# Corleno/Nonstationary_Multivariate_Gaussian_Process

Hardware: AMD Instinct MI355X
Metric: log-posterior evals/sec (N=2048, D=3 nonseparable GP) (higher is better)
Workload: dtype f64

## Files before the change

nonstationary_multivariate_gaussian_process_amd/csrc/nmgp_chol.hip:

```cpp
#include "nmgp_internal.h"
#include <cstring>

namespace nmgpk {

static inline int cdiv_c(long long a, long long b) { return (int)((a + b - 1) / b); }

typedef double v4d __attribute__((ext_vector_type(4)));

#define SY_BM 128
#define SY_BK 16
#define SY_LD (SY_BM + 16)
#define SY_SB 8

__device__ __forceinline__ int clamp_row_pair(int r, int rows) {
    int rc = r < rows - 1 ? r : rows - 2;
    return rc < 0 ? 0 : rc;
}

__device__ __forceinline__ double fast_recip(double p) {
    double x = __builtin_amdgcn_rcp(p);
    double e = fma(-p, x, 1.0);
    x = fma(x, e, x);
    e = fma(-p, x, 1.0);
    x = fma(x, e, x);
    return x;
}

template <int KC, int GC>
__device__ __forceinline__ void potf2_step(double (&a)[16], double (*colbuf)[64], double* pivs, int nb,
                                           int* __restrict__ info, int goff, int r, int g, int tid) {
    constexpr int c = 4 * KC + GC;
    constexpr int NKC = (GC == 3) ? KC + 1 : KC;
    constexpr int NGC = (GC == 3) ? 0 : GC + 1;
    if (c >= nb) return;
    const double* cb = colbuf[c & 1];
    const double piv = cb[c];
    const double mine = cb[r];
    double t[16];
#pragma unroll
    for (int kk = KC; kk < 16; ++kk) t[kk] = cb[4 * kk + g];
    if (tid == 0) {
        pivs[c] = piv;
        if (!(piv > 0.0)) atomicCAS(info, 0, goff + c + 1);
    }
    const double pinv = fast_recip(piv);
    const double f = mine * pinv;
    if (c + 1 < 64) {
        if (NKC < 16) {
            const int cc = 4 * NKC + g;
            const double upd = fma(-f, t[NKC < 16 ? NKC : 15], a[NKC < 16 ? NKC : 15]);
            const bool on = (g == NGC) && (cc <= r);
            if (NKC < 16) a[NKC < 16 ? NKC : 15] = on ? upd : a[NKC < 16 ? NKC : 15];
            if (g == NGC) colbuf[(c + 1) & 1][r] = a[NKC < 16 ? NKC : 15];
        }
        __syncthreads();
    }
#pragma unroll
    for (int kk = KC; kk < 16; ++kk) {
        const int cc = 4 * kk + g;
        const double upd = fma(-f, t[kk], a[kk]);
        bool on = (kk > KC || g > GC) && (cc <= r);
        if (kk == NKC) on = on && (g != NGC);
        a[kk] = on ? upd : a[kk];
    }
}

template <int KC>
__device__ __forceinline__ void potf2_steps4(double (&a)[16], double (*colbuf)[64], double* pivs, int nb,
                                             int* __restrict__ info, int goff, int r, int g, int tid) {
    potf2_step<KC, 0>(a, colbuf, pivs, nb, info, goff, r, g, tid);
    potf2_step<KC, 1>(a, colbuf, pivs, nb, info, goff, r, g, tid);
    potf2_step<KC, 2>(a, colbuf, pivs, nb, info, goff, r, g, tid);
    potf2_step<KC, 3>(a, colbuf, pivs, nb, info, goff, r, g, tid);
}

__device__ __forceinline__ void potf2_body(double* __restrict__ A, int lda, int nb, int* __restrict__ info, int goff, int tid,
                                           double (*colbuf)[64], double* pivs) {
    const int r = tid & 63, g = (tid >> 6) & 3;
    double a[16];
#pragma unroll
    for (int kk = 0; kk < 16; ++kk) {
        const int c = 4 * kk + g;
        double v = (r == c) ? 1.0 : 0.0;
        if (r < nb && c <= r) v = A[(size_t)c * lda + r];
        a[kk] = v;
    }
    if (tid < 64) pivs[tid] = 1.0;
    if (g == 0) colbuf[0][r] = a[0];
    __syncthreads();
#define PF(K) potf2_steps4<K>(a, colbuf, pivs, nb, info, goff, r, g, tid)
    PF(0); PF(1); PF(2); PF(3); PF(4); PF(5); PF(6); PF(7); PF(8); PF(9); PF(10); PF(11); PF(12); PF(13); PF(14); PF(15);
#undef PF
    __syncthreads();
#pragma unroll
    for (int kk = 0; kk < 16; ++kk) {
        const int c = 4 * kk + g;
        if (r < nb && c <= r) A[(size_t)c * lda + r] = a[kk] * rsqrt(pivs[c]);
    }
}

typedef double v2d __attribute__((ext_vector_type(2)));
typedef int v4i __attribute__((ext_vector_type(4)));

__device__ __forceinline__ void syrk_fused_first_block(double* lds, const v4d (&acc)[2][2][2], bool owner, int wj,
                                                       double* __restrict__ C, int ldc, int* __restrict__ info, int goff);

#define SY_SMEM (4 * SY_BK * SY_LD)
#define SCHUR_PATCH (32 * 33)
#define SY_SCHUR_SMEM (8 * SCHUR_PATCH + 6 * 256)
static_assert(SY_SCHUR_SMEM >= SY_SMEM && SY_SCHUR_SMEM * 8 * 2 <= 160 * 1024, "Schur epilogue LDS");

template <int M>
__device__ __forceinline__ double svc_schur_value(double sigma2, int a, int b, bool rc, const double* __restrict__ Lr, double il2,
                                                  const double* __restrict__ Lc, double kv, double nai, double gcb) {
    constexpr int UR = M <= 3 ? 8 : 1;
    const double gra = sigma2 * Lr[a * (a + 1) / 2] * il2;
    double s = 0.0;
#pragma unroll UR
    for (int q = 1; q <= b; ++q) s += Lr[a * (a + 1) / 2 + q] * Lc[b * (b + 1) / 2 + q];
    double v = kv * s;
    if (rc) v += sigma2 * ((a == b ? 1.0 : 0.0) + Lr[a * (a + 1) / 2] * Lr[b * (b + 1) / 2] * il2);
    v += gra * nai * gcb;
    return v;
}

template <int M, bool ALLB>
__device__ __forceinline__ void svc_schur_entries(const SchurEpi& e, double sigma2, int r, const double* __restrict__ Lr, double il2,
                                                  int c, double kv, double nai, const double* gc) {
    constexpr int T = M * (M + 1) / 2;
    constexpr int UR = M <= 3 ? 8 : 1;
    const size_t Ns = (size_t)e.N;
    const double* __restrict__ Lc = e.Lv + (size_t)c * T;
    const double lcc = M <= 4 ? 0.0 : Lc[0];
#pragma unroll UR
    for (int a = 1; a < M; ++a) {
#pragma unroll UR
        for (int b = 1; b <= (ALLB ? a : a - 1); ++b) {
            const double gcb = M <= 4 ? gc[b - 1] : sigma2 * Lc[b * (b + 1) / 2] / (lcc * lcc);
            e.S[((size_t)(b - 1) * Ns + c) * e.ld + ((size_t)(a - 1) * Ns + r)] =
                svc_schur_value<M>(sigma2, a, b, r == c, Lr, il2, Lc, kv, nai, gcb);
        }
    }
}

constexpr int svc_gstride(int M) { return M + 2; }

template <int M>
__device__ __forceinline__ void svc_schur_gtable(const SchurEpi& e, double* lds, int row0, int col0, int tid) {
    constexpr int T = M * (M + 1) / 2, GS = svc_gstride(M);
    if constexpr (M <= 4) {
        double* gt = lds + 8 * SCHUR_PATCH;
        if (tid < 256) {
            const int loc = tid < 128 ? col0 + tid : row0 + tid - 128;
            if (loc < e.N) {
                const double sigma2 = exp(e.tse[0]);
                const double* Lc = e.Lv + (size_t)loc * T;
                const double l00 = Lc[0];
#pragma unroll
                for (int b = 1; b < M; ++b) gt[tid * GS + b - 1] = sigma2 * Lc[b * (b + 1) / 2] / (l00 * l00);
                gt[tid * GS + M - 1] = 1.0 / (l00 * l00);
                gt[tid * GS + M] = e.x[loc];
                gt[tid * GS + M + 1] = e.ell[loc];
            }
        }
        __syncthreads();
    }
}

template <int M>
__device__ __forceinline__ void svc_schur_patch(const SchurEpi& e, double* P, const double* lds, int i0, int j0, int row0, int col0,
                                                int lane) {
    constexpr int T_ = M * (M + 1) / 2, GS = svc_gstride(M);
    constexpr int QU = M <= 3 ? 2 : 1;
    const int N = e.N;
    const size_t Ns = (size_t)N;
    const double sigma2 = exp(e.tse[0]);
    const double* gt = lds + 8 * SCHUR_PATCH;
    const int lo = lane & 31, hi = lane >> 5;
    __builtin_amdgcn_wave_barrier();
#pragma unroll
    for (int pass = 0; pass < 2; ++pass) {
        if (pass == 1 && M == 2) break;
        const int r = (pass == 0 ? i0 : j0) + lo;
        if (r < N) {
            const double* __restrict__ Lr = e.Lv + (size_t)r * T_;
            const double xr = e.x[r], lr = e.ell[r];
            const double xr2 = xr * xr, lr2 = lr * lr;
            const double l00 = Lr[0];
            const double il2 = 1.0 / (l00 * l00);
#pragma unroll QU
            for (int q = 0; q < 16; ++q) {
                const int o = 2 * q + hi;
                const int il = pass == 0 ? lo : o, jl = pass == 0 ? o : lo;
                const int c = (pass == 0 ? j0 : i0) + o;
                if (pass == 0 ? (c > r || c >= N) : (c <= r || c >= N)) continue;
                const double* gc = gt + (pass == 0 ? c - col0 : 128 + c - row0) * GS;
                if (pass == 1 && M == 3) {
                    e.S[(size_t)c * e.ld + (Ns + r)] = P[il * 33 + jl];
                    continue;
                }
                const double xc = M <= 4 ? gc[M] : e.x[c], lc = M <= 4 ? gc[M + 1] : e.ell[c];
                const double dist = (xr2 + xc * xc) - 2.0 * (xr * xc);
                const double Aa = lr2 + lc * lc;
                double kv = sqrt(2.0 * (lr * lc) / Aa) * exp(-dist / Aa);
                if (r == c) kv = NMGP_JITTER + kv;
                const double nai = P[il * 33 + jl];
                if (pass == 0) {
                    svc_schur_entries<M, true>(e, sigma2, r, Lr, il2, c, kv, nai, gc);
                    if (M == 3 && c < r) {
                        const double* Lc = e.Lv + (size_t)c * T_;
                        P[il * 33 + jl] = svc_schur_value<M>(sigma2, 2, 1, false, Lc, gc[M - 1], Lr, kv, nai, gt[(128 + r - row0) * GS]);
                    }
                } else {
                    svc_schur_entries<M, false>(e, sigma2, r, Lr, il2, c, kv, nai, gc);
                }
            }
        }
        __builtin_amdgcn_wave_barrier();
    }
}

template <int M>
__device__ __forceinline__ void svc_schur_yrow(const SchurEpi& e, int i) {
    constexpr int T = M * (M + 1) / 2;
    if (i >= e.N) return;
    const size_t Ns = (size_t)e.N;
    const int n1 = (M - 1) * e.N;
    const double sigma2 = exp(e.tse[0]);
    const double* Li = e.Lv + (size_t)i * T;
    const double l00 = Li[0];
    const double il2 = 1.0 / (l00 * l00);
    const double vi = e.y[i] / l00;
    const double r = vi - (sigma2 * il2) * e.u[i];
#pragma unroll
    for (int a = 1; a < M; ++a) e.S[((size_t)(a - 1) * Ns + i) * e.ld + n1] = e.y[(size_t)a * Ns + i] - Li[a * (a + 1) / 2] * r;
}

template <int SM = 0>
__device__ __forceinline__ void syrk_tile_fast(const double* __restrict__ A, int lda, double* __restrict__ C, int ldc, int K,
                                               int row0, int col0, bool diag, int kt0, bool beta0, int ncw, int yrow,
                                               int nyr, double* sA0, double* sB0, bool skip00 = false,
                                               int* __restrict__ finfo = nullptr, int fgoff = 0, bool mirror = false,
                                               int fresh0 = 0x7fffffff, const SchurEpi* se = nullptr) {
    constexpr int BK = 16;
    constexpr int SBUF = BK * SY_LD;
    const int tid = threadIdx.x, lane = tid & 63, w = tid >> 6;
    const int wi = w & 1, wj = w >> 1;
    const int l15 = lane & 15, l4 = lane >> 4;
    const int rp = tid & 63, cg = tid >> 6;
    const int offA = (cg * lda + row0 + 2 * rp) * 8, offB = (cg * lda + col0 + 2 * rp) * 8;
    const __amdgpu_buffer_rsrc_t rsrc = __builtin_amdgcn_make_buffer_rsrc((void*)A, 0, 0x7fffffff, 0x00020000);
    const int gstep = BK * lda * 8, ghalf = 8 * lda * 8;
    int soff = kt0 * gstep;
    const bool has_y = diag && yrow >= 0;
    const bool ywave = has_y && wi == 0 && wj >= 2;
    const int offY = ((tid & 15) * lda + yrow + (tid >> 4)) * 8;
    double* sY = sB0;
    v4i ra0, ra1, rb0, rb1;
    double ry = 0.0;
    auto gload = [&]() {
        ra0 = __builtin_amdgcn_raw_buffer_load_b128(rsrc, offA, soff, 0);
        ra1 = __builtin_amdgcn_raw_buffer_load_b128(rsrc, offA, soff + ghalf, 0);
        if (!diag) {
            rb0 = __builtin_amdgcn_raw_buffer_load_b128(rsrc, offB, soff, 0);
            rb1 = __builtin_amdgcn_raw_buffer_load_b128(rsrc, offB, soff + ghalf, 0);
        }
        if (has_y && tid < 16 * nyr) {
            typedef int v2i __attribute__((ext_vector_type(2)));
            const v2i t2 = __builtin_amdgcn_raw_buffer_load_b64(rsrc, offY, soff, 0);
            ry = __builtin_bit_cast(double, t2);
        }
        soff += gstep;
    };
    double* wA = sA0 + cg * SY_LD + 2 * rp;
    double* wB = sB0 + cg * SY_LD + 2 * rp;
    auto sstore = [&](int buf) {
        *reinterpret_cast<v4i*>(wA + buf * SBUF) = ra0;
        *reinterpret_cast<v4i*>(wA + buf * SBUF + 8 * SY_LD) = ra1;
        if (!diag) {
            *reinterpret_cast<v4i*>(wB + buf * SBUF) = rb0;
            *reinterpret_cast<v4i*>(wB + buf * SBUF + 8 * SY_LD) = rb1;
        }
        if (has_y && tid < 16 * nyr) sY[buf * 256 + tid] = ry;
    };
    const bool active = !(diag && (wi * 64 + 63 < wj * 32)) && (wj * 32 < ncw) && !(skip00 && wi == 0 && wj < 2);
    const int nk = K / BK;
    gload();
    v4d acc[2][2][2];
    if (active) {
        const int rw0 = __builtin_amdgcn_readfirstlane(row0 + wi * 64);
        const bool wload = !beta0 && rw0 < fresh0;
#pragma unroll
        for (int p = 0; p < 2; ++p) {
            const int i = row0 + wi * 64 + 32 * p + 2 * l15;
            const bool old = i < fresh0;
#pragma unroll
            for (int tj = 0; tj < 2; ++tj)
#pragma unroll
                for (int r = 0; r < 4; ++r) {
                    const int j = col0 + wj * 32 + 2 * (l4 + 4 * r) + tj;
                    double2 c = make_double2(0.0, 0.0);
                    if (wload && old) c = *reinterpret_cast<const double2*>(&C[(size_t)j * ldc + i]);
                    acc[p][0][tj][r] = -c.x;
                    acc[p][1][tj][r] = -c.y;
                }
        }
    }
    if (ywave) {
#pragma unroll
        for (int u = 0; u < 2; ++u)
#pragma unroll
            for (int t = 0; t < 2; ++t)
#pragma unroll
                for (int r = 0; r < 4; ++r) {
                    const int j = col0 + 64 * (wj - 2) + 32 * u + 2 * (l4 + 4 * r) + t;
                    acc[u][0][t][r] = (l15 < nyr && yrow + l15 < fresh0) ? -C[(size_t)j * ldc + yrow + l15] : 0.0;
                }
    }
    sstore(0);
    __syncthreads();
    const double* rA = sA0 + wi * 64 + 2 * l15 + l4 * SY_LD;
    const double* rB = (diag ? sA0 : sB0) + wj * 32 + 2 * l15 + l4 * SY_LD;
    auto compute = [&](int buf) {
        const double* tA = rA + buf * SBUF;
        const double* tB = rB + buf * SBUF;
        v2d fa[2], fb, na[2], nb;
        fa[0] = *reinterpret_cast<const v2d*>(tA);
        fa[1] = *reinterpret_cast<const v2d*>(tA + 32);
        fb = *reinterpret_cast<const v2d*>(tB);
#pragma unroll
        for (int kk = 0; kk < BK / 4; ++kk) {
            if (kk + 1 < BK / 4) {
                na[0] = *reinterpret_cast<const v2d*>(tA + (kk + 1) * 4 * SY_LD);
                na[1] = *reinterpret_cast<const v2d*>(tA + (kk + 1) * 4 * SY_LD + 32);
                nb = *reinterpret_cast<const v2d*>(tB + (kk + 1) * 4 * SY_LD);
            }
#pragma unroll
            for (int tj = 0; tj < 2; ++tj)
#pragma unroll
                for (int p = 0; p < 2; ++p)
#pragma unroll
                    for (int sx = 0; sx < 2; ++sx)
                        acc[p][sx][tj] = __builtin_amdgcn_mfma_f64_16x16x4f64(fb[tj], fa[p][sx], acc[p][sx][tj], 0, 0, 0);
            if (kk + 1 < BK / 4) {
                fa[0] = na[0];
                fa[1] = na[1];
                fb = nb;
            }
        }
    };
    const double* rY = sA0 + 64 * (wj - 2) + 2 * l15 + l4 * SY_LD;
    const int yz = (l15 < nyr) ? yrow + l15 - fresh0 - l4 : 0x7fffffff;
    auto compute_y = [&](int buf, int kb) {
        const double* tB = rY + buf * SBUF;
        const double* ty = sY + buf * 256 + l15 * 16 + l4;
#pragma unroll
        for (int kk = 0; kk < BK / 4; ++kk) {
            const v2d f0 = *reinterpret_cast<const v2d*>(tB + kk * 4 * SY_LD);
            const v2d f1 = *reinterpret_cast<const v2d*>(tB + kk * 4 * SY_LD + 32);
            const double yv = ty[4 * kk];
            const double fy = (kb + 4 * kk >= yz) ? yv : 0.0;
            acc[0][0][0] = __builtin_amdgcn_mfma_f64_16x16x4f64(f0[0], fy, acc[0][0][0], 0, 0, 0);
            acc[0][0][1] = __builtin_amdgcn_mfma_f64_16x16x4f64(f0[1], fy, acc[0][0][1], 0, 0, 0);
            acc[1][0][0] = __builtin_amdgcn_mfma_f64_16x16x4f64(f1[0], fy, acc[1][0][0], 0, 0, 0);
            acc[1][0][1] = __builtin_amdgcn_mfma_f64_16x16x4f64(f1[1], fy, acc[1][0][1], 0, 0, 0);
        }
    };
    for (int kt = kt0; kt < nk; kt += 2) {
        gload();
        if (active) compute(0);
        else if (ywave) compute_y(0, kt * BK);
        sstore(1);
        __syncthreads();
        if (kt + 2 < nk) gload();
        if (active) compute(1);
        else if (ywave) compute_y(1, kt * BK + BK);
        if (kt + 2 < nk) sstore(0);
        __syncthreads();
    }
    if constexpr (SM > 0) {
        svc_schur_gtable<SM>(*se, sA0, row0, col0, tid);
        if (active) {
            double* P = sA0 + w * SCHUR_PATCH;
#pragma unroll
            for (int p = 0; p < 2; ++p) {
#pragma unroll
                for (int sx = 0; sx < 2; ++sx)
#pragma unroll
                    for (int tj = 0; tj < 2; ++tj)
#pragma unroll
                        for (int r = 0; r < 4; ++r) P[(2 * l15 + sx) * 33 + 2 * (l4 + 4 * r) + tj] = -acc[p][sx][tj][r];
                svc_schur_patch<SM>(*se, P, sA0, row0 + wi * 64 + 32 * p, col0 + wj * 32, row0, col0, lane);
            }
        }
        if (diag && wj == 0) svc_schur_yrow<SM>(*se, row0 + wi * 64 + lane);
        return;
    }
    if (ywave && l15 < nyr) {
#pragma unroll
        for (int u = 0; u < 2; ++u)
#pragma unroll
            for (int t = 0; t < 2; ++t)
#pragma unroll
                for (int r = 0; r < 4; ++r) {
                    const int j = col0 + 64 * (wj - 2) + 32 * u + 2 * (l4 + 4 * r) + t;
                    C[(size_t)j * ldc + yrow + l15] = -acc[u][0][t][r];
                }
    }
    const bool fowner = finfo != nullptr && wi == 0 && wj < 2;
    if (active && !fowner) {
#pragma unroll
    for (int p = 0; p < 2; ++p)
#pragma unroll
        for (int tj = 0; tj < 2; ++tj)
#pragma unroll
            for (int r = 0; r < 4; ++r) {
                const int i = row0 + wi * 64 + 32 * p + 2 * l15;
                const int j = col0 + wj * 32 + 2 * (l4 + 4 * r) + tj;
                if (diag && j > i + 1) continue;
                double2 c;
                c.x = -acc[p][0][tj][r];
                c.y = -acc[p][1][tj][r];
                if (diag && j == i + 1) C[(size_t)j * ldc + i + 1] = c.y;
                else *reinterpret_cast<double2*>(&C[(size_t)j * ldc + i]) = c;
            }
    }
    if (mirror && active) {
        double* T = sA0 + w * (32 * 33);
        const int jl = lane & 31, ih = lane >> 5;
#pragma unroll
        for (int p = 0; p < 2; ++p) {
#pragma unroll
            for (int sx = 0; sx < 2; ++sx)
#pragma unroll
                for (int tj = 0; tj < 2; ++tj)
#pragma unroll
                    for (int r = 0; r < 4; ++r) T[(2 * l15 + sx) * 33 + 2 * (l4 + 4 * r) + tj] = -acc[p][sx][tj][r];
            const int rowm = col0 + wj * 32 + jl;
#pragma unroll
            for (int q = 0; q < 16; ++q) {
                const int il = 2 * q + ih;
                const int colm = row0 + wi * 64 + 32 * p + il;
                const double v = T[il * 33 + jl];
                if (colm > rowm) C[(size_t)colm * ldc + rowm] = v;
            }
        }
    }
    if (finfo != nullptr) syrk_fused_first_block(sA0, acc, fowner, wj, C, ldc, finfo, fgoff);
}

template <int NWJ, int BK, int SM = 0>
__device__ __forceinline__ void syrk_tile_body(const double* __restrict__ A, int lda, double* __restrict__ C, int ldc, int mrows,
                                               int ncols, int K, long long bstride, long long cstride, int ktri, int swz,
                                               int nbatch, int bx, int by, int bz0, double* sAb, double* sBb,
                                               int tri_row0 = 0x7fffffff, int tri_k0 = 0, int* __restrict__ finfo = nullptr,
                                               int fistride = 0, int fgoff = 0, const SchurEpi* sep = nullptr) {
    const int nyr = (ktri >> 2) & 31;
    const bool skipq = (ktri & 128) != 0;
    const bool mirror = (ktri & 512) != 0;
    const bool rowmajor = (ktri & 1024) != 0;
    const int yrow = nyr ? mrows : -1;
    (void)rowmajor;
    ktri &= 1;
    const int fresh0 = tri_row0 == 0x7fffffff ? 0x7fffffff : tri_row0 + tri_k0;
    constexpr int NT = 128 * NWJ;
    constexpr int CW = 128 / NWJ;
    constexpr int TJ = CW / 16;
    constexpr int NQ = (64 * BK) / NT;
    constexpr int CGS = NT / 64;
    double (*sA)[BK * SY_LD] = reinterpret_cast<double (*)[BK * SY_LD]>(sAb);
    double (*sB)[BK * SY_LD] = reinterpret_cast<double (*)[BK * SY_LD]>(sBb);
    int bi = bx, bj = by;
    int bz = bz0;
    if (swz) {
        const int t = bx, q = t >> 3;
        const int tiles_pm = swz > 0 ? swz : -swz;
        const long long g = swz > 0 ? ((long long)(q >> 6) * 8 + (t & 7)) * 64 + (q & 63) : (long long)t;
        int idx;
        if (finfo != nullptr) {
            if (g >= (long long)tiles_pm * nbatch) return;
            if (g < nbatch) {
                bz = (int)g;
                idx = 0;
            } else {
                const long long g2 = g - nbatch;
                bz = (int)(g2 / (tiles_pm - 1));
                idx = 1 + (int)(g2 - (long long)bz * (tiles_pm - 1));
            }
        } else {
            bz = (int)(g / tiles_pm);
            if (bz >= nbatch) return;
            idx = (int)(g - (long long)bz * tiles_pm);
        }
        const int gx = (mrows + SY_BM - 1) / SY_BM, gy = (ncols + SY_BM - 1) / SY_BM;
        if (rowmajor) {
            const int tri = gy * (gy + 1) / 2;
            if (idx < tri) {
                int b = (int)((sqrt(8.0 * (double)idx + 1.0) - 1.0) * 0.5);
                while ((b + 1) * (b + 2) / 2 <= idx) ++b;
                while (b * (b + 1) / 2 > idx) --b;
                bi = b;
                bj = idx - b * (b + 1) / 2;
            } else {
                bi = gy + (idx - tri) / gy;
                bj = (idx - tri) % gy;
            }
        } else {
        int c0 = 0, W = 0, cnt = 0;
        for (;; c0 += SY_SB) {
            W = gy - c0 < SY_SB ? gy - c0 : SY_SB;
            cnt = W * (W + 1) / 2 + (gx - c0 - W) * W;
            if (idx < cnt) break;
            idx -= cnt;
        }
        const int tri = W * (W + 1) / 2;
        if (idx < tri) {
            int b = 0;
            while (idx >= W - b) {
                idx -= W - b;
                ++b;
            }
            bj = c0 + b;
            bi = bj + idx;
        } else {
            idx -= tri;
            const int blk = idx / (SY_SB * W), in = idx - blk * (SY_SB * W);
            const int base = c0 + W + blk * SY_SB;
            const int rb = gx - base < SY_SB ? gx - base : SY_SB;
            bj = c0 + in / rb;
            bi = base + in % rb;
        }
        }
    }
    if (bi < bj) return;
    bi = __builtin_amdgcn_readfirstlane(bi);
    bj = __builtin_amdgcn_readfirstlane(bj);
    bz = __builtin_amdgcn_readfirstlane(bz);
    A += (size_t)bz * bstride;
    C += (size_t)bz * cstride;
    SchurEpi se{};
    if constexpr (SM > 0) {
        static_assert(NWJ == 4 && BK == 16, "the Schur epilogue assumes 8 waves of 64 x 32");
        constexpr int T = SM * (SM + 1) / 2;
        se = *sep;
        se.x += (size_t)(bz / se.cps) * se.xstride;
        se.y += (size_t)(bz / se.cps) * se.ystride;
        se.ell += (size_t)bz * se.N;
        se.Lv += (size_t)bz * se.N * T;
        se.tse += (size_t)bz * ((size_t)se.N * (1 + T) + 1);
        se.u += (size_t)bz * se.N;
        se.S += (size_t)bz * se.bstride;
    }
    const bool diag = (bi == bj);
    const int tid = threadIdx.x, lane = tid & 63, w = tid >> 6;
    const int wi = w & 1, wj = w >> 1;
    const int row0 = bi * SY_BM, col0 = bj * SY_BM;
    if constexpr (NWJ == 4 && BK == 16) {
        const int ncw = ncols - col0 >= SY_BM ? SY_BM : ncols - col0;
        if (row0 + SY_BM <= mrows && (ncw == SY_BM || ncw == 64) && col0 + SY_BM <= mrows && (K & 31) == 0 &&
            (long long)(K + 16) * lda * 8 < 0x7fff0000LL) {
            int kt0f = ktri ? row0 / BK : 0;
            if (row0 >= tri_row0) {
                const int z = (row0 - tri_row0 - tri_k0) / BK;
                kt0f = z > 0 ? (z & ~1) : 0;
            }
            syrk_tile_fast<SM>(A, lda, C, ldc, K, row0, col0, diag, kt0f, ktri != 0, ncw, yrow, nyr, &sA[0][0], &sB[0][0],
                               skipq && bi == 0 && bj == 0, (finfo != nullptr && bi == 0 && bj == 0) ? finfo + (size_t)bz * fistride : nullptr,
                               fgoff, mirror, fresh0, &se);
            return;
        }
    }
    const int rp = tid & 63, cg = tid >> 6;
    double2 ra[NQ], rb[NQ];

    const int ri = row0 + 2 * rp, rj = col0 + 2 * rp;
    const int ric = clamp_row_pair(ri, mrows), rjc = clamp_row_pair(rj, mrows);
    const bool ix = ri < mrows, iy = ri + 1 < mrows, jx = rj < mrows, jy = rj + 1 < mrows;
    const bool ish = ix && (ric != ri), jsh = jx && (rjc != rj);
    auto gload = [&](int k0) {
#pragma unroll
        for (int q = 0; q < NQ; ++q) {
            const int kc = k0 + cg + CGS * q;
            const double* colp = A + (size_t)(kc < K ? kc : K - 1) * lda;
            ra[q] = *reinterpret_cast<const double2*>(colp + ric);
            if (!diag) rb[q] = *reinterpret_cast<const double2*>(colp + rjc);
        }
    };
    auto sstore = [&](int buf, int k0) {
#pragma unroll
        for (int q = 0; q < NQ; ++q) {
            const int kl = cg + CGS * q;
            const bool kin = (k0 + kl) < K;
            double2 va, vb;
            va.x = (kin && ix) ? (ish ? ra[q].y : ra[q].x) : 0.0;
            va.y = (kin && iy) ? ra[q].y : 0.0;
            *reinterpret_cast<double2*>(&sA[buf][kl * SY_LD + 2 * rp]) = va;
            if (!diag) {
                vb.x = (kin && jx) ? (jsh ? rb[q].y : rb[q].x) : 0.0;
                vb.y = (kin && jy) ? rb[q].y : 0.0;
                *reinterpret_cast<double2*>(&sB[buf][kl * SY_LD + 2 * rp]) = vb;
            }
        }
    };

    const bool active = !(diag && (wi * 64 + 63 < wj * CW));
    const bool skip00g = skipq && bi == 0 && bj == 0;
    const int nk = (K + BK - 1) / BK;
    int kt0 = ktri ? (row0 / BK) : 0;
    if (row0 >= tri_row0 && row0 - tri_row0 - tri_k0 > 0) kt0 = (row0 - tri_row0 - tri_k0) / BK;
    gload(kt0 * BK);
    v4d acc[TJ][4];
#pragma unroll
    for (int tj = 0; tj < TJ; ++tj)
#pragma unroll
        for (int ti = 0; ti < 4; ++ti)
#pragma unroll
            for (int r = 0; r < 4; ++r) {
                const int i = row0 + wi * 64 + ti * 16 + (lane & 15);
                const int j = col0 + wj * CW + tj * 16 + (lane >> 4) + 4 * r;
                acc[tj][ti][r] = (!ktri && active && i < mrows && j < ncols && i >= j) ? C[(size_t)j * ldc + i] : 0.0;
            }
    if (row0 + SY_BM > fresh0) {
#pragma unroll
        for (int tj = 0; tj < TJ; ++tj)
#pragma unroll
            for (int ti = 0; ti < 4; ++ti)
#pragma unroll
                for (int r = 0; r < 4; ++r)
                    acc[tj][ti][r] = (row0 + wi * 64 + ti * 16 + (lane & 15) >= fresh0) ? 0.0 : acc[tj][ti][r];
    }
    sstore(0, kt0 * BK);
    __syncthreads();
    for (int kt = kt0; kt < nk; ++kt) {
        const int cur = (kt - kt0) & 1;
        if (kt + 1 < nk) gload((kt + 1) * BK);
        if (active) {
            const double* tA = sA[cur] + wi * 64 + (lane & 15) + (lane >> 4) * SY_LD;
            const double* tB = (diag ? sA[cur] : sB[cur]) + wj * CW + (lane & 15) + (lane >> 4) * SY_LD;
            double fa[4], fb[TJ], na[4], nb[TJ];
#pragma unroll
            for (int t = 0; t < 4; ++t) fa[t] = tA[t * 16];
#pragma unroll
            for (int t = 0; t < TJ; ++t) fb[t] = -tB[t * 16];
#pragma unroll
            for (int kk = 0; kk < BK / 4; ++kk) {
                if (kk + 1 < BK / 4) {
#pragma unroll
                    for (int t = 0; t < 4; ++t) na[t] = tA[(kk + 1) * 4 * SY_LD + t * 16];
#pragma unroll
                    for (int t = 0; t < TJ; ++t) nb[t] = -tB[(kk + 1) * 4 * SY_LD + t * 16];
                }
#pragma unroll
                for (int tj = 0; tj < TJ; ++tj)
#pragma unroll
                    for (int ti = 0; ti < 4; ++ti)
                        acc[tj][ti] = __builtin_amdgcn_mfma_f64_16x16x4f64(fb[tj], fa[ti], acc[tj][ti], 0, 0, 0);
                if (kk + 1 < BK / 4) {
#pragma unroll
                    for (int t = 0; t < 4; ++t) fa[t] = na[t];
#pragma unroll
                    for (int t = 0; t < TJ; ++t) fb[t] = nb[t];
                }
            }
        }
        if (kt + 1 < nk) sstore(cur ^ 1, (kt + 1) * BK);
        __syncthreads();
    }
    if constexpr (SM > 0) {
        svc_schur_gtable<SM>(se, sAb, row0, col0, tid);
        if (active) {
            double* P = sAb + w * SCHUR_PATCH;
#pragma unroll
            for (int h = 0; h < 2; ++h) {
#pragma unroll
                for (int tj = 0; tj < TJ; ++tj)
#pragma unroll
                    for (int t2 = 0; t2 < 2; ++t2)
#pragma unroll
                        for (int r = 0; r < 4; ++r)
                            P[(t2 * 16 + (lane & 15)) * 33 + tj * 16 + (lane >> 4) + 4 * r] = acc[tj][2 * h + t2][r];
                svc_schur_patch<SM>(se, P, sAb, row0 + wi * 64 + 32 * h, col0 + wj * CW, row0, col0, lane);
            }
        }
        if (diag && wj == 0) svc_schur_yrow<SM>(se, row0 + wi * 64 + lane);
        return;
    }
    if (active) {
#pragma unroll
        for (int tj = 0; tj < TJ; ++tj)
#pragma unroll
            for (int ti = 0; ti < 4; ++ti)
#pragma unroll
                for (int r = 0; r < 4; ++r) {
                    const int i = row0 + wi * 64 + ti * 16 + (lane & 15);
                    const int j = col0 + wj * CW + tj * 16 + (lane >> 4) + 4 * r;
                    if (i < mrows && j < ncols && i >= j && !(skip00g && i < 64 && j < 64)) C[(size_t)j * ldc + i] = acc[tj][ti][r];
                    if (mirror && i < mrows && j < ncols && i > j) C[(size_t)i * ldc + j] = acc[tj][ti][r];
                }
    }
}

__global__ __launch_bounds__(512, 4) void k_syrk_lower(const double* __restrict__ A, int lda, double* __restrict__ C, int ldc,
                                                        int mrows, int ncols, int K, long long bstride, long long cstride,
                                                        int ktri, int swz, int nbatch, int tri_row0, int tri_k0,
                                                        int* __restrict__ finfo, int fistride, int fgoff) {
    __shared__ __attribute__((aligned(16))) double smem[4 * SY_BK * SY_LD];
    syrk_tile_body<4, SY_BK>(A, lda, C, ldc, mrows, ncols, K, bstride, cstride, ktri, swz, nbatch, blockIdx.x, blockIdx.y,
                             blockIdx.z, smem, smem + 2 * SY_BK * SY_LD, tri_row0, tri_k0, finfo, fistride, fgoff);
}

template <int M>
__global__ __launch_bounds__(512, 4) void k_syrk_schur(const double* __restrict__ A, int lda, int N, long long bstride, int kflags,
                                                        int swz, int nbatch, SchurEpi se) {
    __shared__ __attribute__((aligned(16))) double smem[SY_SCHUR_SMEM];
    syrk_tile_body<4, SY_BK, M>(A, lda, nullptr, 0, N, N, N, bstride, 0, kflags, swz, nbatch, blockIdx.x, blockIdx.y, blockIdx.z,
                                smem, smem + 2 * SY_BK * SY_LD, 0x7fffffff, 0, nullptr, 0, 0, &se);
}

struct Switches {
    enum Panel { kAuto, kFused, kRec, kRl };
    Panel panel = kAuto;
    int fused_max_batch = -1;
    int fused_base = 0;
    int la_max_batch = 16;
    int syrk_small_max = 256;
    const char* step_stamps = nullptr;
};
static const Switches& switches() {
    static const Switches sw = [] {
        Switches w;
        if (const char* e = std::getenv("NMGP_CHOL_PANEL"))
            w.panel = std::strcmp(e, "fused") == 0 ? Switches::kFused
                      : std::strcmp(e, "rec") == 0 ? Switches::kRec : std::strcmp(e, "rl") == 0 ? Switches::kRl : Switches::kAuto;
        if (const char* e = std::getenv("NMGP_CHOL_FUSED_MAX_BATCH")) w.fused_max_batch = std::atoi(e);
        if (const char* e = std::getenv("NMGP_CHOL_FUSED_BASE")) w.fused_base = (std::atoi(e) / 64) * 64;
        if (const char* e = std::getenv("NMGP_CHOL_LA_MAX_BATCH")) w.la_max_batch = std::atoi(e);
        if (const char* e = std::getenv("NMGP_SYRK_SMALL_MAX")) w.syrk_small_max = std::atoi(e);
        w.step_stamps = std::getenv("NMGP_STEP_STAMPS");
        return w;
    }();
    return sw;
}

struct StepStamps {
    long long* dev = nullptr;
    int cap = 0;
    long long* begin(hipStream_t s, int nsteps) {
        if (!switches().step_stamps) return nullptr;
        if (cap < nsteps) {
            if (dev) hipFree(dev);
            if (hipMalloc((void**)&dev, (size_t)nsteps * 16 * sizeof(long long)) != hipSuccess) dev = nullptr;
            cap = dev ? nsteps : 0;
        }
        if (dev) hipMemsetAsync(dev, 0, (size_t)cap * 16 * sizeof(long long), s);
        return dev;
    }
    void dump(hipStream_t s, int nsteps) const {
        if (!switches().step_stamps || !dev) return;
        std::vector<long long> h((size_t)nsteps * 16);
        hipStreamSynchronize(s);
        hipMemcpy(h.data(), dev, h.size() * sizeof(long long), hipMemcpyDeviceToHost);
        if (FILE* f = std::fopen(switches().step_stamps, "w")) {
            for (int k = 0; k < nsteps; ++k) {
                for (int j = 0; j < 9; ++j) std::fprintf(f, "%lld ", h[(size_t)k * 16 + j]);
                std::fprintf(f, "\n");
            }
            std::fclose(f);
        }
    }
};
static StepStamps g_step_stamps;

static constexpr int kNoTriRows = 0x7fffffff;

struct SyrkPlan {
    dim3 grid;
    int swz = 0;
    int kflags = 0;
    int mrows = 0;
    int tiles = 0;
};

static SyrkPlan syrk_plan(int lda, int ldc, int mrows, int ncols, int K, int batch, int ktri, bool compact_only,
                          bool tri_rows = false) {
    SyrkPlan pl;
    int yflag = 0;
    const int nyr = mrows % SY_BM;
    if (!ktri && mrows > SY_BM && nyr >= 1 && nyr <= 16 && ncols % SY_BM == 0 && (K & 31) == 0 &&
        (long long)(K + 16) * lda * 8 < 0x7fff0000LL && (lda & 1) == 0 && (ldc & 1) == 0) {
        yflag = nyr << 2;
        mrows -= nyr;
    }
    pl.mrows = mrows;
    pl.grid = dim3(cdiv_c(mrows, SY_BM), cdiv_c(ncols, SY_BM), batch);
    const int gx = pl.grid.x, gy = pl.grid.y;
// ... 1416 lines not shown
```

Baseline: 1714.

## Add full-subtile Schur epilogue with column table and reversed tile order for odd batches

For M<=3, replaces the per-patch Schur epilogue with a per-wave subtile routine. It precomputes a column table (scaled loadings, x, ell, L entries) in LDS once per tile and keeps row quantities in registers. Accumulator values go through a reshaped 64x17 LDS patch in two halves, and the kernel value is computed inline per column. It also reverses the tile index for odd batches, likely to balance load or locality across concurrently scheduled tiles. This adds code complexity and changes the LDS patch shape.

```diff
diff --git a/nonstationary_multivariate_gaussian_process_amd/csrc/nmgp_chol.hip b/nonstationary_multivariate_gaussian_process_amd/csrc/nmgp_chol.hip
--- a/nonstationary_multivariate_gaussian_process_amd/csrc/nmgp_chol.hip
+++ b/nonstationary_multivariate_gaussian_process_amd/csrc/nmgp_chol.hip
@@ -106,7 +106,7 @@
                                                        double* __restrict__ C, int ldc, int* __restrict__ info, int goff);
 
 #define SY_SMEM (4 * SY_BK * SY_LD)
-#define SCHUR_PATCH (32 * 33)
+#define SCHUR_PATCH (64 * 17)
 #define SY_SCHUR_SMEM (8 * SCHUR_PATCH + 6 * 256)
 static_assert(SY_SCHUR_SMEM >= SY_SMEM && SY_SCHUR_SMEM * 8 * 2 <= 160 * 1024, "Schur epilogue LDS");
 
@@ -236,6 +236,92 @@
     for (int a = 1; a < M; ++a) e.S[((size_t)(a - 1) * Ns + i) * e.ld + n1] = e.y[(size_t)a * Ns + i] - Li[a * (a + 1) / 2] * r;
 }
 
+constexpr int svc_cstride(int M) { return svc_gstride(M) + M * (M + 1) / 2; }
+static_assert(128 * svc_cstride(3) <= 6 * 256, "column table of the full-tile Schur epilogue");
+
+template <int M>
+__device__ __forceinline__ void svc_schur_ctable(const SchurEpi& e, double* lds, int col0, int tid, double sigma2) {
+    constexpr int T = M * (M + 1) / 2, GS = svc_gstride(M), CS = svc_cstride(M);
+    double* ct = lds + 8 * SCHUR_PATCH;
+    if (tid < 128) {
+        const int loc = col0 + tid;
+        const double* Lc = e.Lv + (size_t)loc * T;
+        const double l00 = Lc[0];
+#pragma unroll
+        for (int b = 1; b < M; ++b) ct[tid * CS + b - 1] = sigma2 * Lc[b * (b + 1) / 2] / (l00 * l00);
+        ct[tid * CS + M - 1] = 1.0 / (l00 * l00);
+        ct[tid * CS + M] = e.x[loc];
+        ct[tid * CS + M + 1] = e.ell[loc];
+#pragma unroll
+        for (int t = 0; t < T; ++t) ct[tid * CS + GS + t] = Lc[t];
+    }
+    __syncthreads();
+}
+
+template <int M>
+__device__ __forceinline__ void svc_schur_subtile(const SchurEpi& e, double* P, const double* ct, const v4d (&acc)[2][2][2], int i0,
+                                                  int j0, int col0, int lane, double sigma2) {
+    static_assert(M == 2 || M == 3, "larger M: svc_schur_patch");
+    constexpr int T = M * (M + 1) / 2, GS = svc_gstride(M), CS = svc_cstride(M);
+    const int l15 = lane & 15, l4 = lane >> 4;
+    const size_t Ns = (size_t)e.N, ld = (size_t)e.ld;
+    const int r = i0 + lane;
+    double Lr[T];
+#pragma unroll
+    for (int t = 0; t < T; ++t) Lr[t] = e.Lv[(size_t)r * T + t];
+    const double xr = e.x[r], lr = e.ell[r];
+    const double xr2 = xr * xr, lr2 = lr * lr;
+    const double l00 = Lr[0];
+    const double il2 = 1.0 / (l00 * l00);
+    const double gr1 = sigma2 * Lr[1] / (l00 * l00);
+#pragma unroll
+    for (int h = 0; h < 2; ++h) {
+        const int jh = j0 + 16 * h;
+        __builtin_amdgcn_wave_barrier();
+#pragma unroll
+        for (int p = 0; p < 2; ++p)
+#pragma unroll
+            for (int sx = 0; sx < 2; ++sx)
+#pragma unroll
+                for (int tj = 0; tj < 2; ++tj)
+#pragma unroll
+                    for (int r2 = 0; r2 < 2; ++r2)
+                        P[(32 * p + 2 * l15 + sx) * 17 + 2 * (l4 + 4 * r2) + tj] = -acc[p][sx][tj][2 * h + r2];
+        __builtin_amdgcn_wave_barrier();
+#pragma unroll 2
+        for (int jl = 0; jl < 16; ++jl) {
+            const int c = jh + jl;
+            if (c > r) continue;
+            const double* cc = ct + (c - col0) * CS;
+            const double* Lc = cc + GS;
+            const double xc = cc[M], lc = cc[M + 1];
+            const double dist = (xr2 + xc * xc) - 2.0 * (xr * xc);
+            const double Aa = lr2 + lc * lc;
+            double kv = sqrt(2.0 * (lr * lc) / Aa) * exp(-dist / Aa);
+            if (r == c) kv = NMGP_JITTER + kv;
+            const double nai = P[lane * 17 + jl];
+            double* colp = e.S + ((size_t)c * ld + (size_t)i0);
+#pragma unroll
+            for (int a = 1; a < M; ++a)
+#pragma unroll
+                for (int b = 1; b <= a; ++b)
+                    (colp + ((size_t)(b - 1) * Ns * ld + (size_t)(a - 1) * Ns))[lane] =
+                        svc_schur_value<M>(sigma2, a, b, r == c, Lr, il2, Lc, kv, nai, cc[b - 1]);
+            if (M == 3 && c < r) P[lane * 17 + jl] = svc_schur_value<M>(sigma2, 2, 1, false, Lc, cc[M - 1], Lr, kv, nai, gr1);
+        }
+        if (M == 3) {
+            __builtin_amdgcn_wave_barrier();
+            const int jl = lane & 15, ii = lane >> 4;
+            double* mp = e.S + ((size_t)i0 * ld + Ns + (size_t)jh);
+#pragma unroll 4
+            for (int q = 0; q < 16; ++q) {
+                const int il = 4 * q + ii;
+                if (i0 + il > jh + jl) (mp + (size_t)(4 * q) * ld)[ii * e.ld + jl] = P[il * 17 + jl];
+            }
+        }
+    }
+}
+
 template <int SM = 0>
 __device__ __forceinline__ void syrk_tile_fast(const double* __restrict__ A, int lda, double* __restrict__ C, int ldc, int K,
                                                int row0, int col0, bool diag, int kt0, bool beta0, int ncw, int yrow,
@@ -379,6 +465,16 @@
         __syncthreads();
     }
     if constexpr (SM > 0) {
+        if constexpr (SM <= 3) {
+            const double sigma2 = exp(se->tse[0]);
+            svc_schur_ctable<SM>(*se, sA0, col0, tid, sigma2);
+            if (active)
+                svc_schur_subtile<SM>(*se, sA0 + w * SCHUR_PATCH, sA0 + 8 * SCHUR_PATCH, acc,
+                                      __builtin_amdgcn_readfirstlane(row0 + wi * 64), __builtin_amdgcn_readfirstlane(col0 + wj * 32),
+                                      col0, lane, sigma2);
+            if (diag && wj == 0) svc_schur_yrow<SM>(*se, row0 + wi * 64 + lane);
+            return;
+        }
         svc_schur_gtable<SM>(*se, sA0, row0, col0, tid);
         if (active) {
             double* P = sA0 + w * SCHUR_PATCH;
@@ -491,6 +587,7 @@
             bz = (int)(g / tiles_pm);
             if (bz >= nbatch) return;
             idx = (int)(g - (long long)bz * tiles_pm);
+            if (SM > 0 && (bz & 1) && bz + 8 < nbatch) idx = tiles_pm - 1 - idx;
         }
         const int gx = (mrows + SY_BM - 1) / SY_BM, gy = (ncols + SY_BM - 1) / SY_BM;
         if (rowmajor) {
```

After: 1737 (median of 6 runs). 1.01x the previous value.
